# wenet-e2e/wetts

Measured on AMD Instinct MI355X. Metric: audio samples/sec + RTF @22.05 kHz, VITS-Baker, 1/2/4/8 MI355X, higher is better.
Workload: dtype f32

## Files before the change

wetts_amd/csrc/common.h:

```cpp
#pragma once
#include <hip/hip_runtime.h>
#include <stdint.h>
#include <stdio.h>
#include <string>

#include <string.h>

#include "../../include/wetts_hip.h"

namespace wetts {

void set_error(const char* fmt, ...);

#define WETTS_HIP_CHECK(expr)                                                        \
  do {                                                                               \
    hipError_t _e = (expr);                                                          \
    if (_e != hipSuccess) {                                                          \
      ::wetts::set_error("%s failed: %s (%s:%d)", #expr, hipGetErrorString(_e),      \
                         __FILE__, __LINE__);                                        \
      return WETTS_E_HIP;                                                            \
    }                                                                                \
  } while (0)

static inline bool lds_opt_in(const void* kernel, signed char* state) {
  int dev = 0;
  if (hipGetDevice(&dev) != hipSuccess || dev < 0 || dev >= 64) return false;
  if (state[dev] == 0) {
    const hipError_t e = hipFuncSetAttribute(kernel, hipFuncAttributeMaxDynamicSharedMemorySize, 160 * 1024);
    if (e != hipSuccess) (void)hipGetLastError();
    state[dev] = e == hipSuccess ? 1 : -1;
  }
  return state[dev] > 0;
}

#define WETTS_LAUNCH_CHECK()                                                         \
  do {                                                                               \
    hipError_t _e = hipGetLastError();                                               \
    if (_e != hipSuccess) {                                                          \
      ::wetts::set_error("kernel launch failed: %s (%s:%d)", hipGetErrorString(_e),  \
                         __FILE__, __LINE__);                                        \
      return WETTS_E_HIP;                                                            \
    }                                                                                \
  } while (0)

#define WETTS_REQUIRE(cond, ...)        \
  do {                                  \
    if (!(cond)) {                      \
      ::wetts::set_error(__VA_ARGS__);  \
      return WETTS_E_INVALID;           \
    }                                   \
  } while (0)

#define WETTS_TRY(expr)          \
  do {                           \
    int32_t _r = (expr);         \
    if (_r != WETTS_OK) return _r; \
  } while (0)

constexpr int kConvCK = 16;

enum InAct { IN_NONE = 0, IN_LRELU = 1 };
enum OutAct { OUT_NONE = 0, OUT_RELU = 1, OUT_GELU = 2, OUT_GATE = 3 };
__device__ __forceinline__ float wn_gate(float ta, float sa) { return tanhf(ta) * (1.f / (1.f + expf(-sa))); }

__device__ __forceinline__ float div_small_const(float v, float d, float c) {
  const float q = v * c;
  const float r = __builtin_fmaf(-d, q, v);
  return __builtin_fmaf(r, c, q);
}

__device__ __forceinline__ bool mrf_div_fast(float d) { return d == 3.f || d == 2.f; }
__device__ __forceinline__ float mrf_div(float v, float d, float dinv, bool fast) {
  return fast ? div_small_const(v, d, dinv) : v / d;
}

struct ConvParams {
  const float* x;
  int64_t x_bs, x_cs;
  int Cin, Tin;
  int vec_in;
  int in_rev_base;
  int in_act;
  float in_slope;
  const float* in_mask;
  int64_t in_mask_stride;
  const float* wpk;
  const float* bias;
  const float* bias_b;
  int64_t bias_b_stride;
  int M, N;
  int ktaps, dil, pad;
  int off_lo, span;
  int nchunks;
  float* out;
  int64_t o_bs, o_cs;
  int Tout;
  int up_shift;
  int up, up_pad;
  int out_act;
  const float* out_mask;
  int64_t out_mask_stride;
  const float* res;
  int64_t r_bs, r_cs;
  int accum;
  float out_div;
  int B;
  int tag;
  int k_rows_padded;
  const int64_t* lens;
  int len_mul;
  float* wn_h;
  float* wn_skip;
  const float* wn_mask;
  int64_t wn_mask_stride;
  int wn_H, wn_last, wn_first;
};

inline ConvParams conv_io(const float* x, int Cin, int T, float* out, int Cout, int B) {
  ConvParams p;
  memset(&p, 0, sizeof(p));
  p.x = x;
  p.x_bs = (int64_t)Cin * T;
  p.x_cs = T;
  p.Tin = T;
  p.in_rev_base = -1;
  p.in_act = IN_NONE;
  p.in_slope = 0.f;
  p.out = out;
  p.o_bs = (int64_t)Cout * T;
  p.o_cs = T;
  p.Tout = T;
  p.out_act = OUT_NONE;
  p.out_div = 1.f;
  p.B = B;
  return p;
}

struct PackedConv {
  float* wpk = nullptr;
  const float* bias = nullptr;
  int M = 0, Cin = 0, ktaps = 0, dil = 1, pad = 0;
  int up = 0, up_pad = 0;
  int Cout = 0;
  int k_orig = 0;
  int off_lo = 0, span = 0, nchunks = 0;
  int gate_H = 0;
};

int32_t pack_conv_weight(const float* w_dev, const float* bias_dev, int Cout, int Cin, int k,
                         int dil, int pad, int transposed, int up, hipStream_t stream,
                         PackedConv* out, int rev_in = 0, int gate_H = 0);
void free_packed(PackedConv* pc);

int32_t launch_conv(const PackedConv& pc, ConvParams p, hipStream_t stream);
bool pw_gemm_eligible(const PackedConv& pc, const ConvParams& p);
int32_t launch_pw_gemm(const PackedConv& pc, const ConvParams& p, hipStream_t stream, int variant);
int32_t launch_conv_group(const PackedConv* const* pcs, const ConvParams* ps, int n, hipStream_t stream,
                          int* launches = nullptr);

int conv_variant();
void set_conv_variant(int v);
int32_t launch_conv_small(const ConvParams& p, hipStream_t stream, bool* taken);
struct SmallConvScope {
  explicit SmallConvScope(int max_tiles);
  ~SmallConvScope();
  int prev;
};

inline int cdiv(int a, int b) { return (a + b - 1) / b; }
inline int64_t align_up(int64_t v, int64_t a) { return (v + a - 1) / a * a; }

inline int device_cus() {
  static int cus = 0;
  if (cus == 0) {
    int dev = 0, n = 0;
    cus = (hipGetDevice(&dev) == hipSuccess &&
           hipDeviceGetAttribute(&n, hipDeviceAttributeMultiprocessorCount, dev) == hipSuccess && n > 0) ? n : 256;
  }
  return cus;
}

}
```

wetts_amd/csrc/conv_mfma.hip:

```cpp
#include <stdlib.h>

#include "common.h"

namespace wetts {

typedef float f32x16 __attribute__((ext_vector_type(16)));
typedef float f32x4v __attribute__((ext_vector_type(4)));
constexpr int kBufRsrcDword3 = 0x00020000;

__device__ __forceinline__ float lrelu2(float x, float slope) {
  const float m = x * slope;
  float r;
  asm("v_max_f32 %0, %1, %2" : "=v"(r) : "v"(x), "v"(m));
  return r;
}

__global__ void pack_conv_weight_kernel(const float* __restrict__ w, float* __restrict__ out,
                                        int M, int Cin, int Cout, int k, int ktaps, int up,
                                        int transposed, int rev_in, int gate_H, int G, int64_t total) {
  int64_t idx = (int64_t)blockIdx.x * blockDim.x + threadIdx.x;
  if (idx >= total) return;
  int s = (int)(idx & 3);
  int lane = (int)((idx >> 2) & 63);
  int64_t rest = idx >> 8;
// ... 299 lines not shown
  for (int i = 0; i < MB; ++i) a_nxt[i] = abase[i][0];
#pragma unroll
  for (int i = 0; i < MB; ++i) a_alt[i] = a_nxt[i];

  load_chunk(0);
  store_chunk(buf0);
  __syncthreads();

  const int half = lane >> 5;
  const int bcol0 = wn * (32 * NB) + (lane & 31) - p.pad - p.off_lo + sh;
  int g = 0;
  for (int c = 0; c < p.nchunks; ++c) {
    const float* cur = (c & 1) ? buf1 : buf0;
    const bool more = (c + 1) < p.nchunks;
    if (more) load_chunk(c + 1);
    for (int tap = 0; tap < p.ktaps; ++tap) {
      const int coff = bcol0 + tap * p.dil;
#pragma unroll
      for (int hp = 0; hp < 2; ++hp) {
        float4 a_cur[MB];
        ++g;
        if (hp == 0) {
#pragma unroll
          for (int i = 0; i < MB; ++i) a_cur[i] = a_nxt[i];
#pragma unroll
          for (int i = 0; i < MB; ++i) a_alt[i] = abase[i][(int64_t)g * 64];
        } else {
#pragma unroll
          for (int i = 0; i < MB; ++i) a_cur[i] = a_alt[i];
#pragma unroll
          for (int i = 0; i < MB; ++i) a_nxt[i] = abase[i][(int64_t)g * 64];
        }
        __builtin_amdgcn_sched_barrier(0);
        const float* brow0 = cur + (hp * 8 + half) * W + coff;
        float bv[2][NB];
#pragma unroll
        for (int s = 0; s < 4; ++s) {
#pragma unroll
          for (int j = 0; j < NB; ++j) bv[s & 1][j] = brow0[s * 2 * W + 32 * j];
#pragma unroll
          for (int i = 0; i < MB; ++i) {
            const float av = s == 0 ? a_cur[i].x : s == 1 ? a_cur[i].y : s == 2 ? a_cur[i].z
                                                                                 : a_cur[i].w;
#pragma unroll
            for (int j = 0; j < NB; ++j)
              acc[i][j] = __builtin_amdgcn_mfma_f32_32x32x2f32(av, bv[s & 1][j], acc[i][j], 0, 0, 0);
          }
        }
      }
    }
    if (more) store_chunk((c & 1) ? buf0 : buf1);
    __syncthreads();
  }

  const int64_t ob = (int64_t)b * p.o_bs;
  const int64_t rb = (int64_t)b * p.r_bs;
  const float* bb = p.bias_b ? p.bias_b + (int64_t)b * p.bias_b_stride : nullptr;
  const float* omask = p.out_mask ? p.out_mask + (int64_t)b * p.out_mask_stride : nullptr;
  if (EPI == 5) {
    const int gH = p.M >> 1;
#pragma unroll
    for (int i = 0; i < MB; ++i) {
      const int mrow0 = mtile * MT + (wm * MB + i) * 32 + 4 * half;
      float bt[8], bs[8], ut[8], us[8];
#pragma unroll
      for (int q = 0; q < 8; ++q) {
        const int r = 2 * q;
        const int gi = min(mrow0 + (r & 3) + 8 * (r >> 2), p.M - 2) >> 1;
        bt[q] = p.bias ? p.bias[gi] : 0.f;
        bs[q] = p.bias ? p.bias[gH + gi] : 0.f;
        ut[q] = bb ? bb[gi] : 0.f;
        us[q] = bb ? bb[gH + gi] : 0.f;
      }
#pragma unroll
      for (int r = 0; r < 16; r += 2) {
        const int row = mrow0 + (r & 3) + 8 * (r >> 2);
        if (row >= p.M) continue;
        const int gi = row >> 1, q = r >> 1;
        float b0 = bt[q], b1 = bs[q], u0 = ut[q], u1 = us[q];
        if (full_tile) { b0 += u0; b1 += u1; u0 = u1 = 0.f; }
#pragma unroll
        for (int j = 0; j < NB; ++j) {
          const int col = n0 + wn * (32 * NB) + j * 32 + (lane & 31);
          if (col < N)
            p.out[ob + (int64_t)gi * p.o_cs + col] = wn_gate((acc[i][j][r] + b0) + u0, (acc[i][j][r + 1] + b1) + u1);
        }
      }
    }
    return;
  }
  if (EPI != 0 && full_tile) {
    char* obase = reinterpret_cast<char*>(p.out + ob + (int64_t)wrow0 * p.o_cs + wcol0);
    const unsigned ocs4 = (unsigned)p.o_cs * 4u;
    const unsigned olane = (unsigned)(4 * half) * ocs4 + (unsigned)(lane & 31) * 4u;
    float bia[MB][16];
#pragma unroll
    for (int i = 0; i < MB; ++i)
#pragma unroll
      for (int r = 0; r < 16; ++r) bia[i][r] = 0.f;
    if (p.bias) {
      const float* bp = p.bias + wrow0 + 4 * half;
#pragma unroll
      for (int i = 0; i < MB; ++i)
#pragma unroll
        for (int r = 0; r < 16; ++r) bia[i][r] = bp[i * 32 + (r & 3) + 8 * (r >> 2)];
    }
    if (bb) {
      const float* bp = bb + wrow0 + 4 * half;
#pragma unroll
      for (int i = 0; i < MB; ++i)
#pragma unroll
        for (int r = 0; r < 16; ++r) bia[i][r] += bp[i * 32 + (r & 3) + 8 * (r >> 2)];
    }
    float om[NB];
#pragma unroll
    for (int j = 0; j < NB; ++j) om[j] = EPI == 4 ? omask[wcol0 + 32 * j + (lane & 31)] : 1.f;
    auto store_all = [&](auto fin) {
#pragma unroll
      for (int i = 0; i < MB; ++i) {
#pragma unroll
        for (int r = 0; r < 16; ++r) {
          const int rloc = i * 32 + (r & 3) + 8 * (r >> 2);
          const unsigned roff = (unsigned)rloc * ocs4 + olane;
#pragma unroll
          for (int j = 0; j < NB; ++j) {
            float v = fin(acc[i][j][r] + bia[i][r]);
            if (EPI == 4) v *= om[j];
            *reinterpret_cast<float*>(obase + (roff + 128u * j)) = v;
          }
        }
      }
    };
    if (EPI == 2) {
      const float dv = p.out_div, dinv = 1.f / p.out_div;
      if (mrf_div_fast(dv)) store_all([=](float v) { return div_small_const(v, dv, dinv); });
      else store_all([=](float v) { return v / dv; });
    } else {
      store_all([](float v) { return v; });
    }
    return;
  }
  if (EPI == 3) {
    const int sh = p.up_shift, um = p.up - 1;
    char* obase = reinterpret_cast<char*>(p.out + ob);
    const unsigned ocs4 = (unsigned)p.o_cs * 4u;
    float bia[MB][16];
#pragma unroll
    for (int i = 0; i < MB; ++i)
#pragma unroll
      for (int r = 0; r < 16; ++r) {
        const int row = wrow0 + i * 32 + (r & 3) + 8 * (r >> 2) + 4 * half;
        bia[i][r] = (p.bias && row < p.M) ? p.bias[row >> sh] : 0.f;
      }
    if (sh >= 2 && (p.up_pad & 3) == 0 && (Tout & 3) == 0 && (p.M & 3) == 0) {
#pragma unroll
      for (int i = 0; i < MB; ++i) {
#pragma unroll
        for (int q = 0; q < 4; ++q) {
          const int row = wrow0 + i * 32 + 8 * q + 4 * half;
          const int co = row >> sh, ph = row & um;
          const unsigned rowoff = (unsigned)co * ocs4;
#pragma unroll
          for (int j = 0; j < NB; ++j) {
            const int col = wcol0 + 32 * j + (lane & 31);
            const int t = (col << sh) + ph - p.up_pad;
            if (row < p.M && col < N && t >= 0 && t < Tout) {
              f32x4v v;
              v.x = acc[i][j][4 * q] + bia[i][4 * q];
              v.y = acc[i][j][4 * q + 1] + bia[i][4 * q + 1];
              v.z = acc[i][j][4 * q + 2] + bia[i][4 * q + 2];
              v.w = acc[i][j][4 * q + 3] + bia[i][4 * q + 3];
              *reinterpret_cast<f32x4v*>(obase + (rowoff + (unsigned)t * 4u)) = v;
            }
          }
        }
      }
      return;
    }
#pragma unroll
    for (int i = 0; i < MB; ++i) {
#pragma unroll
      for (int r = 0; r < 16; ++r) {
        const int row = wrow0 + i * 32 + (r & 3) + 8 * (r >> 2) + 4 * half;
        const int co = row >> sh, ph = row & um;
        const unsigned rowoff = (unsigned)co * ocs4;
#pragma unroll
        for (int j = 0; j < NB; ++j) {
          const int col = wcol0 + 32 * j + (lane & 31);
          const int t = (col << sh) + ph - p.up_pad;
          if (row < p.M && col < N && t >= 0 && t < Tout)
            *reinterpret_cast<float*>(obase + (rowoff + (unsigned)t * 4u)) = acc[i][j][r] + bia[i][r];
        }
      }
    }
    return;
  }
#pragma unroll
  for (int i = 0; i < MB; ++i) {
    const int mrow0 = mtile * MT + (wm * MB + i) * 32 + 4 * half;
#pragma unroll
    for (int j = 0; j < NB; ++j) {
      const int col = n0 + wn * (32 * NB) + j * 32 + (lane & 31);
      if (col >= N) continue;
#pragma unroll
      for (int r = 0; r < 16; ++r) {
        const int row = mrow0 + (r & 3) + 8 * (r >> 2);
        if (row >= p.M) continue;
        int co = row, t = col;
        if (p.up > 0) {
          co = row / p.up;
          t = col * p.up + (row - co * p.up) - p.up_pad;
          if (t < 0 || t >= Tout) continue;
        }
        float v = acc[i][j][r];
        if (p.bias) v += p.bias[co];
        if (bb) v += bb[co];
        if (p.wn_skip) {
          const int64_t hb = (int64_t)b * p.wn_H * p.Tout + t;
          if (!p.wn_last && row < p.wn_H) {
            float* hp = p.wn_h + hb + (int64_t)row * p.Tout;
            *hp = (*hp + v) * p.wn_mask[(int64_t)b * p.wn_mask_stride + t];
          } else {
            float* sp = p.wn_skip + hb + (int64_t)(p.wn_last ? row : row - p.wn_H) * p.Tout;
            *sp = p.wn_first ? v : *sp + v;
          }
          continue;
        }
        if (p.out_act == OUT_RELU) v = v > 0.f ? v : 0.f;
        if (p.out_act == OUT_GELU) v = 0.5f * v * (1.f + erff(v * 0.70710678118654752f));
        if (omask) v *= omask[t];
        float* dst = p.out + ob + (int64_t)co * p.o_cs + t;
        if (!pre_res) {
          if (p.res) v += p.res[rb + (int64_t)co * p.r_cs + t];
          if (p.accum) v += *dst;
        }
        if (p.out_div != 1.f) v = mrf_div(v, p.out_div, 1.f / p.out_div, mrf_div_fast(p.out_div));
        *dst = v;
      }
    }
  }
}

template <int MB, int NB, int WM, int WN, int EPI = 0, bool MRF = false, bool FAST = false>
__global__ __launch_bounds__(256) __attribute__((amdgpu_waves_per_eu((MB * NB >= 4 && WN < 4) ? 3 : 1)))
void conv_mfma_kernel(const ConvParams p) {
  conv_mfma_body<MB, NB, WM, WN, EPI, FAST>(p, blockIdx.x);
}

constexpr int kConvGroupMax = 3;
struct ConvGroupParams {
  ConvParams p[kConvGroupMax];
  int first[kConvGroupMax + 1];
  int n;
};
template <int MB, int NB, int WM, int WN, int EPI>
__global__ __launch_bounds__(256) __attribute__((amdgpu_waves_per_eu((MB * NB >= 4 && WN < 4) ? 3 : 1)))
void conv_mfma_group_kernel(const ConvGroupParams gp) {
  const int bid = blockIdx.x;
  int j = 0;
  if (gp.n > 1 && bid >= gp.first[1]) j = 1;
  if (gp.n > 2 && bid >= gp.first[2]) j = 2;
  conv_mfma_body<MB, NB, WM, WN, EPI, true>(gp.p[j], bid - gp.first[j]);
}



static bool conv_fast_ok(const ConvParams& p);

static int g_conv_variant = -1;

int conv_variant() {
  if (g_conv_variant < 0) {
    const char* e = getenv("WETTS_CONV_VARIANT");
    g_conv_variant = e ? atoi(e) : 0;
  }
  return g_conv_variant;
}
void set_conv_variant(int v) { g_conv_variant = v; }

template <int MB, int NB, int WM, int WN>
static int32_t launch_cfg(const ConvParams& p, hipStream_t stream) {
  constexpr int MT = 32 * MB * WM, NT = 32 * NB * WN;
  int ntiles = cdiv(p.N, NT), mtiles = cdiv(p.M, MT);
  int64_t blocks = (int64_t)ntiles * mtiles * p.B;
  if (blocks <= 0) return WETTS_OK;
  WETTS_REQUIRE(blocks < (1ll << 31), "conv grid too large");
  const bool fast = conv_fast_ok(p);
  const size_t lds = (size_t)2 * kConvCK *
                     (fast ? (conv_has_fixed_stride(NT) ? conv_fixed_stride(NT) : ((NT + p.span + 3 + 3) & ~3)) : NT + p.span) *
                     sizeof(float);
  const dim3 grid((unsigned)blocks), blk(256);
  const bool plain = p.up == 0 && p.out_act == OUT_NONE && p.out_mask == nullptr && p.wn_skip == nullptr;
  if (p.out_act == OUT_GATE) {
    if (fast)
      hipLaunchKernelGGL((conv_mfma_kernel<MB, NB, WM, WN, 5, false, true>), grid, blk, lds, stream, p);
    else
      hipLaunchKernelGGL((conv_mfma_kernel<MB, NB, WM, WN, 5, false>), grid, blk, lds, stream, p);
  } else if (p.up > 0 && p.up_shift >= 0 && p.out_act == OUT_NONE && !p.out_mask && !p.res && !p.accum &&
      !p.bias_b && p.out_div == 1.f) {
    if (fast)
      hipLaunchKernelGGL((conv_mfma_kernel<MB, NB, WM, WN, 3, false, true>), grid, blk, lds, stream, p);
    else
      hipLaunchKernelGGL((conv_mfma_kernel<MB, NB, WM, WN, 3, false>), grid, blk, lds, stream, p);
  } else if (p.up == 0 && p.out_act == OUT_NONE && p.out_mask && !p.res && !p.accum && p.out_div == 1.f) {
    if (fast)
      hipLaunchKernelGGL((conv_mfma_kernel<MB, NB, WM, WN, 4, false, true>), grid, blk, lds, stream, p);
    else
      hipLaunchKernelGGL((conv_mfma_kernel<MB, NB, WM, WN, 4, false>), grid, blk, lds, stream, p);
  } else if (plain && p.tag && fast) {
    if (p.out_div == 1.f)
      hipLaunchKernelGGL((conv_mfma_kernel<MB, NB, WM, WN, 1, true, true>), grid, blk, lds, stream, p);
    else
      hipLaunchKernelGGL((conv_mfma_kernel<MB, NB, WM, WN, 2, true, true>), grid, blk, lds, stream, p);
  } else if (plain && p.tag) {
    if (p.out_div == 1.f)
      hipLaunchKernelGGL((conv_mfma_kernel<MB, NB, WM, WN, 1, true>), grid, blk, lds, stream, p);
    else
      hipLaunchKernelGGL((conv_mfma_kernel<MB, NB, WM, WN, 2, true>), grid, blk, lds, stream, p);
  } else if (plain && p.out_div == 1.f && fast) {
    hipLaunchKernelGGL((conv_mfma_kernel<MB, NB, WM, WN, 1, false, true>), grid, blk, lds, stream, p);
  } else if (plain && p.out_div == 1.f) {
    hipLaunchKernelGGL((conv_mfma_kernel<MB, NB, WM, WN, 1, false>), grid, blk, lds, stream, p);
  } else if (plain) {
    hipLaunchKernelGGL((conv_mfma_kernel<MB, NB, WM, WN, 2, false>), grid, blk, lds, stream, p);
  } else if (fast) {
    hipLaunchKernelGGL((conv_mfma_kernel<MB, NB, WM, WN, 0, false, true>), grid, blk, lds, stream, p);
  } else {
    hipLaunchKernelGGL((conv_mfma_kernel<MB, NB, WM, WN, 0, false>), grid, blk, lds, stream, p);
  }
  WETTS_LAUNCH_CHECK();
  return WETTS_OK;
}

static int32_t prepare_conv(const PackedConv& pc, ConvParams& p) {
  p.wpk = pc.wpk;
  p.bias = pc.bias;
  p.M = pc.M;
  p.Cin = pc.Cin;
  p.ktaps = pc.ktaps;
  p.dil = pc.dil;
  p.pad = pc.pad;
  p.off_lo = pc.off_lo;
  p.span = pc.span;
  p.nchunks = pc.nchunks;
  p.up = pc.up;
  p.up_pad = pc.up_pad;
  p.up_shift = -1;
  for (int q = 0; q < 16; ++q)
    if (pc.up == (1 << q)) p.up_shift = q;
  WETTS_REQUIRE(pc.wpk != nullptr, "conv weight not packed");
  WETTS_REQUIRE((p.out_act == OUT_GATE) == (pc.gate_H > 0), "gate epilogue and interleaved packing go together");
  WETTS_REQUIRE(p.out_act != OUT_GATE || (!p.res && !p.accum && !p.out_mask && p.out_div == 1.f && !p.wn_skip && pc.up == 0),
                "gate epilogue: plain store only");
  if (pc.ktaps == 1 && pc.up == 0 && p.in_mask && p.in_mask == p.out_mask &&
      p.in_mask_stride == p.out_mask_stride && p.out_act == OUT_NONE)
    p.in_mask = nullptr;
  WETTS_REQUIRE(p.span <= 128, "conv receptive field too wide (span %d > 128)", p.span);
  if (p.up > 0) {
    p.N = p.Tin + p.ktaps - 1;
  } else {
    p.N = p.Tout;
  }
  return WETTS_OK;
}

static bool conv_fast_ok(const ConvParams& p) {
  return p.in_mask == nullptr && p.in_rev_base < 0 && (p.Cin % kConvCK) == 0 && (p.x_cs & 3) == 0 &&
         (p.x_bs & 3) == 0 && (p.Tin & 3) == 0 && p.span <= 125 && (reinterpret_cast<uintptr_t>(p.x) & 15) == 0 &&
         ((int64_t)p.Cin * p.x_cs) < (1ll << 29) && (p.lens == nullptr || (p.len_mul & 3) == 0);
}

template <int MB, int NB, int WM, int WN>
static int32_t launch_group_cfg(ConvGroupParams& gp, int max_span, hipStream_t stream) {
  constexpr int MT = 32 * MB * WM, NT = 32 * NB * WN;
  int64_t total = 0;
  for (int j = 0; j < gp.n; ++j) {
    gp.first[j] = (int)total;
    total += (int64_t)cdiv(gp.p[j].N, NT) * cdiv(gp.p[j].M, MT) * gp.p[j].B;
  }
  gp.first[gp.n] = (int)total;
  WETTS_REQUIRE(total > 0 && total < (1ll << 31), "conv group grid size");
  const size_t lds = (size_t)2 * kConvCK * (conv_has_fixed_stride(NT) ? conv_fixed_stride(NT) : ((NT + max_span + 3 + 3) & ~3)) *
                     sizeof(float);
  hipLaunchKernelGGL((conv_mfma_group_kernel<MB, NB, WM, WN, 1>), dim3((unsigned)total), dim3(256), lds, stream, gp);
  WETTS_LAUNCH_CHECK();
  return WETTS_OK;
}

int32_t launch_conv_group(const PackedConv* const* pcs, const ConvParams* ps, int n, hipStream_t stream,
                          int* launches) {
  if (launches) *launches = n;
  if (n <= 0) return WETTS_OK;
  ConvGroupParams gp;
  memset(&gp, 0, sizeof(gp));
  bool ok = n >= 2 && n <= kConvGroupMax && conv_variant() == 0;
  int order[kConvGroupMax] = {0, 1, 2};
  if (ok) {
    for (int a = 0; a < n; ++a)
      for (int b = a + 1; b < n; ++b)
        if (pcs[order[b]]->ktaps > pcs[order[a]]->ktaps) { int t = order[a]; order[a] = order[b]; order[b] = t; }
  }
  int max_span = 0;
  for (int j = 0; j < n && ok; ++j) {
    gp.p[j] = ps[order[j]];
    WETTS_TRY(prepare_conv(*pcs[order[j]], gp.p[j]));
    const ConvParams& q = gp.p[j];
    ok = q.up == 0 && q.out_act == OUT_NONE && q.out_mask == nullptr && q.out_div == 1.f && q.tag && conv_fast_ok(q) &&
         q.M == gp.p[0].M && q.N == gp.p[0].N && q.B == gp.p[0].B && q.Cin == gp.p[0].Cin && q.lens == gp.p[0].lens;
    if (q.span > max_span) max_span = q.span;
  }
  gp.n = n;
  if (ok) {
    const ConvParams& q = gp.p[0];
    const int64_t cols = (int64_t)q.N * q.B;
    auto nblk = [&](int mt, int nt) { return (int64_t)cdiv(q.M, mt) * cdiv(q.N, nt) * q.B; };
    if (q.M >= 128 && cols >= 4096 && nblk(128, 128) >= 384) {
      if (launches) *launches = 1;
      return launch_group_cfg<1, 4, 4, 1>(gp, max_span, stream);
    }
    if (q.M > 32 && q.M < 128 && cols >= 8192 && nblk(64, 256) >= 384) {
      if (launches) *launches = 1;
      return launch_group_cfg<1, 4, 2, 2>(gp, max_span, stream);
    }
  }
  for (int j = 0; j < n; ++j) WETTS_TRY(launch_conv(*pcs[j], ps[j], stream));
  return WETTS_OK;
}

int32_t launch_conv(const PackedConv& pc, ConvParams p, hipStream_t stream) {
  WETTS_TRY(prepare_conv(pc, p));
  if (conv_variant() == 0 && p.lens == nullptr) {
    bool taken = false;
    WETTS_TRY(launch_conv_small(p, stream, &taken));
    if (taken) return WETTS_OK;
  }
  {
    const int v = conv_variant();
    if ((v == 0 || (v >= 7 && v <= 9)) && pw_gemm_eligible(pc, p)) return launch_pw_gemm(pc, p, stream, v);
  }
  const int64_t cols = (int64_t)p.N * p.B;
  switch (conv_variant()) {
    case 2: return launch_cfg<1, 2, 4, 1>(p, stream);
    case 3: return launch_cfg<1, 4, 2, 2>(p, stream);
    case 4: return launch_cfg<1, 2, 2, 2>(p, stream);
    case 5: return launch_cfg<1, 1, 2, 2>(p, stream);
    case 6: return launch_cfg<1, 4, 4, 1>(p, stream);
    default: break;
  }
  auto nblk = [&](int mt, int nt) { return (int64_t)cdiv(p.M, mt) * cdiv(p.N, nt) * p.B; };
  constexpr int64_t kFill = 384;
  if (p.M >= 128 && cols >= 4096) {
    const int64_t n128 = nblk(128, 128);
    const int kCUs = device_cus();
    if (n128 >= 4 * kCUs) return launch_cfg<1, 4, 4, 1>(p, stream);
    auto cost = [&](int64_t blocks, int area, double eff) {
      return (blocks < kCUs ? 4.0 : 1.0) * (double)((blocks + kCUs - 1) / kCUs) * area / eff;
    };
    const double c128 = cost(n128, 128 * 128, 1.18), c64w = cost(nblk(64, 128), 64 * 128, 1.07),
                 c64 = cost(nblk(64, 64), 64 * 64, 1.0);
    if (c128 <= c64w && c128 <= c64) return launch_cfg<1, 4, 4, 1>(p, stream);
    if (c64w <= c64) return launch_cfg<1, 2, 2, 2>(p, stream);
    return launch_cfg<1, 1, 2, 2>(p, stream);
  }
  if (p.M > 32 && cols >= 8192) {
    if (nblk(64, 256) >= kFill) return launch_cfg<1, 4, 2, 2>(p, stream);
    return launch_cfg<1, 1, 2, 2>(p, stream);
  }
  if (p.M <= 32 && cols >= 8192 && p.ktaps >= 5) return launch_cfg<1, 4, 1, 4>(p, stream);
  if (p.M <= 32 && cols >= 8192) return launch_cfg<1, 2, 1, 4>(p, stream);
  return launch_cfg<1, 1, 2, 2>(p, stream);
}

}
```

wetts_amd/csrc/kernels.h:

```cpp
#pragma once
#include "common.h"

namespace wetts {

int32_t k_embed_mask(const int64_t* ids, const int64_t* lengths, const float* emb, int n_vocab,
                     int B, int H, int T, float* x_out, float* mask_out, int32_t* status,
                     hipStream_t s);

int32_t k_layernorm(const float* a, const float* add, const float* gamma, const float* beta,
                    const float* res, const float* mask, int gelu, int B, int C, int T, float* out,
                    hipStream_t s);

struct DdsFusedParams {
  const float* x;
  float* out;
  const float* mask;
  const float *sep_w[3], *sep_b[3], *n1g[3], *n1b[3], *n2g[3], *n2b[3];
  const float* wpk[3];
  const float* bias[3];
  int B, C, T, G;
};
bool dds_fused_supported(int mode, int C, int Cw, int nchunks, int B, int T);
int32_t k_dds_fused(DdsFusedParams p, hipStream_t s);
int32_t k_dwconv(const float* x, const float* mask, const float* w, const float* bias, int k,
                 int dil, int B, int C, int T, float* out, hipStream_t s, int Tvalid = 0);

int32_t k_cond_linear(const float* g, const float* W, const float* bias, int B, int Cout, int K,
                      float* out, hipStream_t s);

int32_t k_gather_rows(const int64_t* idx, const float* table, int n_rows, int B, int C, float* out,
                      int32_t* status, hipStream_t s);

int32_t k_add_bias_b(float* x, const float* v, int B, int C, int T, hipStream_t s);
int32_t k_add_bias_b_mask(float* x, const float* v, const float* mask, int B, int C, int T,
                          hipStream_t s);
int32_t k_scale(const float* a, float scale, int64_t n, float* out, hipStream_t s);

int32_t k_convflow_pre(const float* z, int ch0, const float* w, const float* bias, const float* g,
                       int B, int C, int T, float* out, hipStream_t s);

int32_t k_spline_inverse(float* z, int ch0, int ch1, const float* h, const float* mask,
                         int num_bins, float tail_bound, float inv_sqrt_div, int B, int T,
                         int32_t* status, hipStream_t s);

int32_t k_affine_reverse(const float* z, int ch, const float* m, const float* logs, int param_idx,
                         const float* mask, int B, int T, float* logw, hipStream_t s);

int32_t k_gate(const float* a, int B, int H, int T, float* out, hipStream_t s);

int32_t k_wn_update(const float* rs, float* h, float* skip, const float* mask, int last, int first,
                    int B, int H, int T, hipStream_t s);

int32_t k_coupling_flip(const float* xin, const float* m, const float* mask, int B, int C, int T,
                        float* out, hipStream_t s);

int32_t k_conv_post_tanh(const float* x, const float* w, int k, int B, int C, int T, float* out,
                         hipStream_t s, const int64_t* lens = nullptr, int len_mul = 0);

int32_t k_durations_to_lengths(const float* logw, const float* mask, float length_scale, int B,
                               int T, float* w_ceil, float* cum, int64_t* y_lengths,
                               int32_t* status, hipStream_t s);

int32_t k_frame_index(const float* cum, const int64_t* y_lengths, int B, int Tx, int Ty,
                      int32_t* frame2phone, float* y_mask, hipStream_t s);
int32_t k_expand_prior(const float* stats, const int32_t* frame2phone, const float* eps,
                       int64_t eps_bs, int64_t eps_cs, float noise_scale, int B, int C, int Tx, int Ty, float* m_exp,
                       float* logs_exp, float* z_p, hipStream_t s);
int32_t k_attn_path(const int32_t* frame2phone, int B, int Tx, int Ty, float* attn, hipStream_t s);

int32_t k_audio_to_int16(const float* audio, const int64_t* lengths, int B, int64_t L, int16_t* pcm,
                         hipStream_t s);

int32_t k_vocos_pad(const float* z, int64_t z_bs, int64_t z_cs, const float* mask,
                    int64_t mask_stride, int B, int C, int L, float* out, hipStream_t s, int Fs = 0);
int32_t k_vocos_spec(const float* spec, int B, int half, int F, float* ri, hipStream_t s, int64_t ri_bs = 0);
int32_t k_istft_basis(int n_fft, float* w, hipStream_t s, double inv_scale = 0.0);
bool k_convnext_dwln(const float* x, const float* w, const float* wb, const float* gamma, const float* beta, int B, int C,
                     int T, int Tvalid, float* out, hipStream_t s, int32_t* rc);
int32_t k_istft_ola(const float* frames, int B, int n_fft, int hop, int F, float* audio,
                    hipStream_t s, int Fs = 0, int envelope = 1);
int32_t k_scale_rows(const float* a, const float* scale, int rows, int cols, float* out,
                     hipStream_t s);

int32_t k_flip_half(const float* x, const float* mask, int B, int C, int T, float* x0, float* x0m,
                    hipStream_t s);
int32_t k_mono_split(const float* x, const float* mask, int B, int C, int T, float sc, float* x0, float* x0m,
                     hipStream_t s);
int32_t k_mono_coupling(const float* x, const float* m, const float* mask, int B, int C, int T, float sc, float* out,
                        hipStream_t s);
int32_t k_coupling_fwd_flip(const float* x, const float* m, const float* mask, int B, int C, int T, float* out,
                            hipStream_t s);
int32_t k_mono_coupling_fwd(const float* x, const float* m, const float* mask, int B, int C, int T, int residual,
                            float* out, hipStream_t s);
int32_t k_seq_mask(const int64_t* lengths, int B, int T_in, int Tp, float* mask, float* mask_out, hipStream_t s);
int32_t k_posterior_sample(const float* stats, const float* eps, const float* mask, int B, int C, int T, int Tp,
                           float* z, float* m_out, float* logs_out, hipStream_t s);
int32_t k_copy_rows(const float* src, int64_t src_stride, int cols_src, float* dst, int64_t dst_stride, int cols_dst,
                    int64_t rows, hipStream_t s);
int32_t k_add(const float* a, const float* b, int64_t n, float* out, hipStream_t s);

int32_t k_rel_attention(const float* q, const float* k, const float* v, int64_t qkv_batch_stride,
                        const float* mask, const float* emb_rel_k, const float* emb_rel_v,
                        int window, int B, int n_heads, int dk, int T, float* scores, float* out,
                        hipStream_t s);

int64_t attn_score_elems(int window, int dk, int B, int n_heads, int T);

int32_t k_randn(float* out, int64_t n, uint64_t seed, uint64_t offset, hipStream_t s);
int32_t k_mask_rows(const float* x, const float* mask, int B, int C, int T, float* out,
                    hipStream_t s);

int32_t k_mas(const float* neg_cent, const int32_t* t_ys, const int32_t* t_xs, int B, int Ty,
              int Tx, int32_t* path, float* values, hipStream_t s);

int32_t k_align_scores(const float* z_p, const float* stats, int B, int I, int Tx, int Ty, float* neg_cent,
                       hipStream_t s);
int32_t k_align_lengths(const int64_t* x_lengths, const int64_t* y_lengths, int B, int Tx, int Ty, int32_t* t_xs,
                        int32_t* t_ys, int32_t* status, hipStream_t s);
int32_t k_path_to_durations(const int32_t* path, const int32_t* t_ys, const int32_t* t_xs, int B, int Tx, int Ty,
                            float* w, float* cum, int32_t* frame2phone, float* attn, hipStream_t s);
int32_t k_counts_to_lengths(const int64_t* counts, const float* mask, int B, int T, float* w_ceil, float* cum,
                            int64_t* y_lengths, int32_t* status, hipStream_t s);

}
```

wetts_amd/csrc/kernels.hip:

```cpp
#include "kernels.h"

namespace wetts {

static inline dim3 grid1d(int64_t n, int threads) {
  return dim3((unsigned)((n + threads - 1) / threads));
}

__global__ void embed_mask_kernel(const int64_t* __restrict__ ids,
                                  const int64_t* __restrict__ lengths,
                                  const float* __restrict__ emb, int n_vocab, int B, int H, int T,
                                  float scale, float* __restrict__ x_out,
                                  float* __restrict__ mask_out, int32_t* __restrict__ status) {
  int64_t idx = (int64_t)blockIdx.x * blockDim.x + threadIdx.x;
  int64_t total = (int64_t)B * H * T;
  if (idx >= total) return;
  int t = (int)(idx % T);
  int c = (int)((idx / T) % H);
  int b = (int)(idx / ((int64_t)T * H));
  bool valid = (int64_t)t < lengths[b];
  float v = 0.f;
  if (valid) {
    int64_t id = ids[(int64_t)b * T + t];
    if (id < 0 || id >= n_vocab) {
      if (status && c == 0) atomicOr(status, WETTS_STATUS_PHONE_ID_RANGE);
// ... 499 lines not shown
int32_t k_affine_reverse(const float* z, int ch, const float* m, const float* logs, int param_idx,
                         const float* mask, int B, int T, float* logw, hipStream_t s) {
  if (B * T == 0) return WETTS_OK;
  hipLaunchKernelGGL(affine_reverse_kernel, grid1d((int64_t)B * T, 256), dim3(256), 0, s, z, ch, m,
                     logs, param_idx, mask, B, T, logw);
  WETTS_LAUNCH_CHECK();
  return WETTS_OK;
}

__global__ void gate_kernel(const float* __restrict__ a, int B, int H, int T,
                            float* __restrict__ out) {
  int64_t idx = (int64_t)blockIdx.x * blockDim.x + threadIdx.x;
  int64_t total = (int64_t)B * H * T;
  if (idx >= total) return;
  int64_t ht = (int64_t)H * T;
  int64_t b = idx / ht, r = idx % ht;
  float ta = a[b * 2 * ht + r];
  float sa = a[b * 2 * ht + ht + r];
  out[idx] = tanhf(ta) * (1.f / (1.f + expf(-sa)));
}

int32_t k_gate(const float* a, int B, int H, int T, float* out, hipStream_t s) {
  int64_t n = (int64_t)B * H * T;
  if (n == 0) return WETTS_OK;
  hipLaunchKernelGGL(gate_kernel, grid1d(n, 256), dim3(256), 0, s, a, B, H, T, out);
  WETTS_LAUNCH_CHECK();
  return WETTS_OK;
}

__global__ void wn_update_kernel(const float* __restrict__ rs, float* __restrict__ h,
                                 float* __restrict__ skip, const float* __restrict__ mask, int last,
                                 int first, int B, int H, int T) {
  int64_t idx = (int64_t)blockIdx.x * blockDim.x + threadIdx.x;
  int64_t total = (int64_t)B * H * T;
  if (idx >= total) return;
  int64_t ht = (int64_t)H * T;
  int64_t b = idx / ht, r = idx % ht;
  int t = (int)(r % T);
  float sk;
  if (!last) {
    float res = rs[b * 2 * ht + r];
    sk = rs[b * 2 * ht + ht + r];
    h[idx] = (h[idx] + res) * mask[b * T + t];
  } else {
    sk = rs[idx];
  }
  skip[idx] = first ? sk : skip[idx] + sk;
}

int32_t k_wn_update(const float* rs, float* h, float* skip, const float* mask, int last, int first,
                    int B, int H, int T, hipStream_t s) {
  int64_t n = (int64_t)B * H * T;
  if (n == 0) return WETTS_OK;
  hipLaunchKernelGGL(wn_update_kernel, grid1d(n, 256), dim3(256), 0, s, rs, h, skip, mask, last,
                     first, B, H, T);
  WETTS_LAUNCH_CHECK();
  return WETTS_OK;
}

__global__ void coupling_flip_kernel(const float* __restrict__ xin, const float* __restrict__ m,
                                     const float* __restrict__ mask, int B, int C, int T,
                                     float* __restrict__ out) {
  int64_t idx = (int64_t)blockIdx.x * blockDim.x + threadIdx.x;
  int64_t total = (int64_t)B * C * T;
  if (idx >= total) return;
  int t = (int)(idx % T);
  int c = (int)((idx / T) % C);
  int b = (int)(idx / ((int64_t)T * C));
  const int half = C / 2;
  float v = xin[((int64_t)b * C + (C - 1 - c)) * T + t];
  if (c >= half) v = (v - m[((int64_t)b * half + (c - half)) * T + t]) * mask[(int64_t)b * T + t];
  out[idx] = v;
}

int32_t k_coupling_flip(const float* xin, const float* m, const float* mask, int B, int C, int T,
                        float* out, hipStream_t s) {
  int64_t n = (int64_t)B * C * T;
  if (n == 0) return WETTS_OK;
  hipLaunchKernelGGL(coupling_flip_kernel, grid1d(n, 256), dim3(256), 0, s, xin, m, mask, B, C, T,
                     out);
  WETTS_LAUNCH_CHECK();
  return WETTS_OK;
}

__global__ __launch_bounds__(256) void conv_post_tanh_kernel(const float* __restrict__ x,
                                                             const float* __restrict__ w, int k,
                                                             int B, int C, int T,
                                                             float* __restrict__ out,
                                                             const int64_t* __restrict__ lens, int len_mul) {
  extern __shared__ float wsh[];
  for (int i = threadIdx.x; i < C * k; i += blockDim.x) wsh[i] = w[i];
  __syncthreads();
  const int per_b = (T + 3) / 4;
  int64_t idx = (int64_t)blockIdx.x * blockDim.x + threadIdx.x;
  if (idx >= (int64_t)B * per_b) return;
  const int b = (int)(idx / per_b);
  const int t0 = (int)(idx % per_b) * 4;
  const int pad = (k - 1) / 2;
  float acc[4] = {0.f, 0.f, 0.f, 0.f};
  const float* xb = x + (int64_t)b * C * T;
  const int Tb = lens ? min((int)lens[b] * len_mul, T) : T;
  if (t0 >= Tb) {
#pragma unroll
    for (int o = 0; o < 4; ++o)
      if (t0 + o < T) out[(int64_t)b * T + t0 + o] = 0.f;
    return;
  }
  if (k == 7 && (T & 3) == 0 && t0 >= 4 && t0 + 8 <= Tb && (C & 3) == 0 &&
      (reinterpret_cast<uintptr_t>(xb) & 15) == 0) {
    for (int c = 0; c < C; c += 4) {
      float4 v[4][3];
#pragma unroll
      for (int u = 0; u < 4; ++u) {
        const float4* xr4 = reinterpret_cast<const float4*>(xb + (int64_t)(c + u) * T + (t0 - 4));
        v[u][0] = xr4[0];
        v[u][1] = xr4[1];
        v[u][2] = xr4[2];
      }
#pragma unroll
      for (int u = 0; u < 4; ++u) {
        const float raw[10] = {v[u][0].y, v[u][0].z, v[u][0].w, v[u][1].x, v[u][1].y,
                               v[u][1].z, v[u][1].w, v[u][2].x, v[u][2].y, v[u][2].z};
        float win[10];
#pragma unroll
        for (int i = 0; i < 10; ++i) win[i] = raw[i] > 0.f ? raw[i] : raw[i] * 0.01f;
#pragma unroll
        for (int j = 0; j < 7; ++j) {
          const float wv = wsh[(c + u) * 7 + j];
#pragma unroll
          for (int o = 0; o < 4; ++o) acc[o] += wv * win[o + j];
        }
      }
    }
  } else
  for (int c = 0; c < C; ++c) {
    const float* xr = xb + (int64_t)c * T;
    float win[4 + 15];
    for (int i = 0; i < 3 + k; ++i) {
      int tt = t0 - pad + i;
      float v = (tt >= 0 && tt < Tb) ? xr[tt] : 0.f;
      win[i] = v > 0.f ? v : v * 0.01f;
    }
    for (int j = 0; j < k; ++j) {
      float wv = wsh[c * k + j];
#pragma unroll
      for (int o = 0; o < 4; ++o) acc[o] += wv * win[o + j];
    }
  }
#pragma unroll
  for (int o = 0; o < 4; ++o)
    if (t0 + o < T) out[(int64_t)b * T + t0 + o] = (t0 + o < Tb) ? tanhf(acc[o]) : 0.f;
}

template <int K>
__global__ __launch_bounds__(256) void conv_post_tanh_small_kernel(const float* __restrict__ x,
                                                                   const float* __restrict__ w, int B,
                                                                   int C, int T, float* __restrict__ out) {
  constexpr int TL = 32, CG = 8, MAXC = 8;
  __shared__ float red[CG][TL + 1];
  const int tl = threadIdx.x % TL, cg = threadIdx.x / TL;
  const int tblocks = (T + TL - 1) / TL;
  const int b = blockIdx.x / tblocks;
  const int t = (blockIdx.x % tblocks) * TL + tl;
  constexpr int pad = (K - 1) / 2;
  const float* xb = x + (int64_t)b * C * T;
  float win[MAXC][K], wv[MAXC][K];
#pragma unroll
  for (int j = 0; j < MAXC; ++j) {
    const int c = cg + CG * j;
    const int cc = c < C ? c : 0;
#pragma unroll
    for (int i = 0; i < K; ++i) {
      const int tt = t - pad + i;
      const bool ok = c < C && tt >= 0 && tt < T;
      win[j][i] = xb[(int64_t)cc * T + (ok ? tt : 0)];
      wv[j][i] = ok ? w[cc * K + i] : 0.f;
    }
  }
  float acc = 0.f;
#pragma unroll
  for (int j = 0; j < MAXC; ++j)
#pragma unroll
    for (int i = 0; i < K; ++i) {
      const float v = win[j][i];
      acc += wv[j][i] * (v > 0.f ? v : v * 0.01f);
    }
  red[cg][tl] = acc;
  __syncthreads();
  if (cg == 0 && t < T) {
    float tot = 0.f;
#pragma unroll
    for (int q = 0; q < CG; ++q) tot += red[q][tl];
    out[(int64_t)b * T + t] = tanhf(tot);
  }
}

int32_t k_conv_post_tanh(const float* x, const float* w, int k, int B, int C, int T, float* out,
                         hipStream_t s, const int64_t* lens, int len_mul) {
  WETTS_REQUIRE(k <= 15, "conv_post kernel size %d unsupported", k);
  int64_t n = (int64_t)B * ((T + 3) / 4);
  if (n == 0) return WETTS_OK;
  if (k == 7 && C <= 64 && n <= 64 * 256 && !lens) {
    hipLaunchKernelGGL(conv_post_tanh_small_kernel<7>, dim3((unsigned)(B * cdiv(T, 32))), dim3(256), 0, s, x, w,
                       B, C, T, out);
    WETTS_LAUNCH_CHECK();
    return WETTS_OK;
  }
  hipLaunchKernelGGL(conv_post_tanh_kernel, grid1d(n, 256), dim3(256), (size_t)C * k * 4, s, x, w,
                     k, B, C, T, out, lens, len_mul);
  WETTS_LAUNCH_CHECK();
  return WETTS_OK;
}

__global__ __launch_bounds__(64) void durations_kernel(const float* __restrict__ logw,
                                                       const float* __restrict__ mask,
                                                       float length_scale, int B, int T,
                                                       float* __restrict__ w_ceil,
                                                       float* __restrict__ cum,
                                                       int64_t* __restrict__ y_lengths,
                                                       int32_t* __restrict__ status) {
  const int b = blockIdx.x, lane = threadIdx.x;
  float carry = 0.f;
  for (int t0 = 0; t0 < T; t0 += 64) {
    int t = t0 + lane;
    float wc = 0.f;
    if (t < T) {
      float w = expf(logw[(int64_t)b * T + t]) * mask[(int64_t)b * T + t] * length_scale;
      wc = ceilf(w);
      w_ceil[(int64_t)b * T + t] = wc;
    }
    float v = wc;
#pragma unroll
    for (int off = 1; off < 64; off <<= 1) {
      float n = __shfl_up(v, off, 64);
      if (lane >= off) v += n;
    }
    v += carry;
    if (t < T) cum[(int64_t)b * T + t] = v;
    carry = __shfl(v, 63, 64);
  }
  if (lane == 0) {
    float tot = carry < 1.f ? 1.f : carry;
    if (!(tot <= 9.0e15f)) {
      if (status) atomicOr(status, WETTS_STATUS_DURATION_NONFINITE);
      tot = 1.f;
    }
    y_lengths[b] = (int64_t)tot;
  }
}

int32_t k_durations_to_lengths(const float* logw, const float* mask, float length_scale, int B,
                               int T, float* w_ceil, float* cum, int64_t* y_lengths,
                               int32_t* status, hipStream_t s) {
  if (B == 0) return WETTS_OK;
  hipLaunchKernelGGL(durations_kernel, dim3(B), dim3(64), 0, s, logw, mask, length_scale, B, T,
                     w_ceil, cum, y_lengths, status);
  WETTS_LAUNCH_CHECK();
  return WETTS_OK;
}

__global__ void frame_index_kernel(const float* __restrict__ cum,
                                   const int64_t* __restrict__ y_lengths, int B, int Tx, int Ty,
                                   int32_t* __restrict__ f2p, float* __restrict__ y_mask) {
  int idx = blockIdx.x * blockDim.x + threadIdx.x;
  if (idx >= B * Ty) return;
  int ty = idx % Ty, b = idx / Ty;
  bool valid = (int64_t)ty < y_lengths[b];
  int res = -1;
  if (valid) {
    const float* cr = cum + (int64_t)b * Tx;
    int lo = 0, hi = Tx;
    float fy = (float)ty;
    while (lo < hi) {
      int mid = (lo + hi) >> 1;
      if (cr[mid] > fy) hi = mid; else lo = mid + 1;
    }
    if (lo < Tx) res = lo;
  }
  f2p[idx] = res;
  y_mask[idx] = valid ? 1.f : 0.f;
}

int32_t k_frame_index(const float* cum, const int64_t* y_lengths, int B, int Tx, int Ty,
                      int32_t* frame2phone, float* y_mask, hipStream_t s) {
  if (B * Ty == 0) return WETTS_OK;
  hipLaunchKernelGGL(frame_index_kernel, grid1d((int64_t)B * Ty, 256), dim3(256), 0, s, cum,
                     y_lengths, B, Tx, Ty, frame2phone, y_mask);
  WETTS_LAUNCH_CHECK();
  return WETTS_OK;
}

__global__ void expand_prior_kernel(const float* __restrict__ stats,
                                    const int32_t* __restrict__ f2p, const float* __restrict__ eps,
                                    int64_t eps_bs, int64_t eps_cs, float noise_scale, int B, int C, int Tx, int Ty,
                                    float* __restrict__ m_exp, float* __restrict__ logs_exp,
                                    float* __restrict__ z_p) {
  int64_t idx = (int64_t)blockIdx.x * blockDim.x + threadIdx.x;
  int64_t total = (int64_t)B * C * Ty;
  if (idx >= total) return;
  int ty = (int)(idx % Ty);
  int c = (int)((idx / Ty) % C);
  int b = (int)(idx / ((int64_t)Ty * C));
  int tx = f2p[(int64_t)b * Ty + ty];
  float m = 0.f, ls = 0.f;
  if (tx >= 0) {
    m = stats[((int64_t)b * 2 * C + c) * Tx + tx];
    ls = stats[((int64_t)b * 2 * C + C + c) * Tx + tx];
  }
  if (m_exp) m_exp[idx] = m;
  if (logs_exp) logs_exp[idx] = ls;
  const float e = eps[(int64_t)b * eps_bs + (int64_t)c * eps_cs + ty];
  z_p[idx] = m + e * expf(ls) * noise_scale;
}

int32_t k_expand_prior(const float* stats, const int32_t* frame2phone, const float* eps,
                       int64_t eps_bs, int64_t eps_cs, float noise_scale, int B, int C, int Tx, int Ty, float* m_exp,
                       float* logs_exp, float* z_p, hipStream_t s) {
  int64_t n = (int64_t)B * C * Ty;
  if (n == 0) return WETTS_OK;
  hipLaunchKernelGGL(expand_prior_kernel, grid1d(n, 256), dim3(256), 0, s, stats, frame2phone, eps,
                     eps_bs, eps_cs, noise_scale, B, C, Tx, Ty, m_exp, logs_exp, z_p);
  WETTS_LAUNCH_CHECK();
  return WETTS_OK;
}

__global__ void attn_path_kernel(const int32_t* __restrict__ f2p, int B, int Tx, int Ty,
                                 float* __restrict__ attn) {
  int64_t idx = (int64_t)blockIdx.x * blockDim.x + threadIdx.x;
  int64_t total = (int64_t)B * Ty * Tx;
  if (idx >= total) return;
  int tx = (int)(idx % Tx);
  int64_t bty = idx / Tx;
  attn[idx] = (f2p[bty] == tx) ? 1.f : 0.f;
}

int32_t k_attn_path(const int32_t* frame2phone, int B, int Tx, int Ty, float* attn, hipStream_t s) {
  int64_t n = (int64_t)B * Ty * Tx;
  if (n == 0) return WETTS_OK;
  hipLaunchKernelGGL(attn_path_kernel, grid1d(n, 256), dim3(256), 0, s, frame2phone, B, Tx, Ty,
                     attn);
  WETTS_LAUNCH_CHECK();
  return WETTS_OK;
}

__global__ __launch_bounds__(256) void audio_to_int16_kernel(const float* __restrict__ audio,
                                                             const int64_t* __restrict__ lengths,
                                                             int64_t L, int16_t* __restrict__ pcm) {
  __shared__ float red[4];
  const int b = blockIdx.x;
  const float* a = audio + (int64_t)b * L;
  int64_t n = lengths ? lengths[b] : L;
  if (n > L) n = L;
  float mx = 0.f;
  for (int64_t i = threadIdx.x; i < n; i += blockDim.x) mx = fmaxf(mx, fabsf(a[i]));
#pragma unroll
// ... 428 lines not shown
```

Baseline: 52.49 million.

## Add cost-model tile choice for upsampling convs and staged-tile conv_post kernel

Moves conv tile selection into a reusable function and gives transposed/upsampling convs their own cost model across 128x128, 128x64 and 64x128 tiles, instead of always taking 128x128 when the block count is large. It also adds an LDS double-buffered conv_post+tanh kernel that stages four channels at a time with halos. That kernel only runs when variant==2, and no caller in view passes that value. The vectorized upsample store now also checks output alignment, which guards against misaligned float4 writes.

```diff
diff --git a/wetts_amd/csrc/common.h b/wetts_amd/csrc/common.h
--- a/wetts_amd/csrc/common.h
+++ b/wetts_amd/csrc/common.h
@@ -160,6 +160,7 @@
 
 int conv_variant();
 void set_conv_variant(int v);
+int conv_tile_choice(int M, int N, int B, int ktaps, int up, int cus);
 int32_t launch_conv_small(const ConvParams& p, hipStream_t stream, bool* taken);
 struct SmallConvScope {
   explicit SmallConvScope(int max_tiles);
diff --git a/wetts_amd/csrc/conv_mfma.hip b/wetts_amd/csrc/conv_mfma.hip
--- a/wetts_amd/csrc/conv_mfma.hip
+++ b/wetts_amd/csrc/conv_mfma.hip
@@ -475,7 +475,8 @@
         const int row = wrow0 + i * 32 + (r & 3) + 8 * (r >> 2) + 4 * half;
         bia[i][r] = (p.bias && row < p.M) ? p.bias[row >> sh] : 0.f;
       }
-    if (sh >= 2 && (p.up_pad & 3) == 0 && (Tout & 3) == 0 && (p.M & 3) == 0) {
+    if (sh >= 2 && (p.up_pad & 3) == 0 && (Tout & 3) == 0 && (p.M & 3) == 0 && (p.o_cs & 3) == 0 &&
+        (reinterpret_cast<uintptr_t>(obase) & 15) == 0) {
 #pragma unroll
       for (int i = 0; i < MB; ++i) {
 #pragma unroll
@@ -589,6 +590,8 @@
 
 
 static bool conv_fast_ok(const ConvParams& p);
+
+constexpr double kUpEff128 = 1.18, kUpEff128n = 1.10, kUpEff64w = 1.07;
 
 static int g_conv_variant = -1;
 
@@ -761,7 +764,6 @@
     const int v = conv_variant();
     if ((v == 0 || (v >= 7 && v <= 9)) && pw_gemm_eligible(pc, p)) return launch_pw_gemm(pc, p, stream, v);
   }
-  const int64_t cols = (int64_t)p.N * p.B;
   switch (conv_variant()) {
     case 2: return launch_cfg<1, 2, 4, 1>(p, stream);
     case 3: return launch_cfg<1, 4, 2, 2>(p, stream);
@@ -770,28 +772,47 @@
     case 6: return launch_cfg<1, 4, 4, 1>(p, stream);
     default: break;
   }
-  auto nblk = [&](int mt, int nt) { return (int64_t)cdiv(p.M, mt) * cdiv(p.N, nt) * p.B; };
+  switch (conv_tile_choice(p.M, p.N, p.B, p.ktaps, p.up, device_cus())) {
+    case 128128: return launch_cfg<1, 4, 4, 1>(p, stream);
+    case 128064: return launch_cfg<1, 2, 4, 1>(p, stream);
+    case 64256: return launch_cfg<1, 4, 2, 2>(p, stream);
+    case 64128: return launch_cfg<1, 2, 2, 2>(p, stream);
+    case 32512: return launch_cfg<1, 4, 1, 4>(p, stream);
+    case 32256: return launch_cfg<1, 2, 1, 4>(p, stream);
+    default: return launch_cfg<1, 1, 2, 2>(p, stream);
+  }
+}
+
+int conv_tile_choice(int M, int N, int B, int ktaps, int up, int cus) {
+  const int64_t cols = (int64_t)N * B;
+  auto nblk = [&](int mt, int nt) { return (int64_t)cdiv(M, mt) * cdiv(N, nt) * B; };
   constexpr int64_t kFill = 384;
-  if (p.M >= 128 && cols >= 4096) {
+  if (M >= 128 && cols >= 4096) {
     const int64_t n128 = nblk(128, 128);
-    const int kCUs = device_cus();
-    if (n128 >= 4 * kCUs) return launch_cfg<1, 4, 4, 1>(p, stream);
+    const int kCUs = cus;
     auto cost = [&](int64_t blocks, int area, double eff) {
       return (blocks < kCUs ? 4.0 : 1.0) * (double)((blocks + kCUs - 1) / kCUs) * area / eff;
     };
+    if (up > 0) {
+      const double u128 = cost(n128, 128 * 128, kUpEff128), u128n = cost(nblk(128, 64), 128 * 64, kUpEff128n),
+                   u64w = cost(nblk(64, 128), 64 * 128, kUpEff64w);
+      if (u128 <= u128n && u128 <= u64w) return 128128;
+      return u128n <= u64w ? 128064 : 64128;
+    }
+    if (n128 >= 4 * kCUs) return 128128;
     const double c128 = cost(n128, 128 * 128, 1.18), c64w = cost(nblk(64, 128), 64 * 128, 1.07),
                  c64 = cost(nblk(64, 64), 64 * 64, 1.0);
-    if (c128 <= c64w && c128 <= c64) return launch_cfg<1, 4, 4, 1>(p, stream);
-    if (c64w <= c64) return launch_cfg<1, 2, 2, 2>(p, stream);
-    return launch_cfg<1, 1, 2, 2>(p, stream);
-  }
-  if (p.M > 32 && cols >= 8192) {
-    if (nblk(64, 256) >= kFill) return launch_cfg<1, 4, 2, 2>(p, stream);
-    return launch_cfg<1, 1, 2, 2>(p, stream);
-  }
-  if (p.M <= 32 && cols >= 8192 && p.ktaps >= 5) return launch_cfg<1, 4, 1, 4>(p, stream);
-  if (p.M <= 32 && cols >= 8192) return launch_cfg<1, 2, 1, 4>(p, stream);
-  return launch_cfg<1, 1, 2, 2>(p, stream);
-}
-
-}
+    if (c128 <= c64w && c128 <= c64) return 128128;
+    if (c64w <= c64) return 64128;
+    return 64064;
+  }
+  if (M > 32 && cols >= 8192) {
+    if (nblk(64, 256) >= kFill) return 64256;
+    return 64064;
+  }
+  if (M <= 32 && cols >= 8192 && ktaps >= 5) return 32512;
+  if (M <= 32 && cols >= 8192) return 32256;
+  return 64064;
+}
+
+}
diff --git a/wetts_amd/csrc/kernels.h b/wetts_amd/csrc/kernels.h
--- a/wetts_amd/csrc/kernels.h
+++ b/wetts_amd/csrc/kernels.h
@@ -55,7 +55,7 @@
                         float* out, hipStream_t s);
 
 int32_t k_conv_post_tanh(const float* x, const float* w, int k, int B, int C, int T, float* out,
-                         hipStream_t s, const int64_t* lens = nullptr, int len_mul = 0);
+                         hipStream_t s, const int64_t* lens = nullptr, int len_mul = 0, int variant = 0);
 
 int32_t k_durations_to_lengths(const float* logw, const float* mask, float length_scale, int B,
                                int T, float* w_ceil, float* cum, int64_t* y_lengths,
diff --git a/wetts_amd/csrc/kernels.hip b/wetts_amd/csrc/kernels.hip
--- a/wetts_amd/csrc/kernels.hip
+++ b/wetts_amd/csrc/kernels.hip
@@ -675,6 +675,90 @@
     if (t0 + o < T) out[(int64_t)b * T + t0 + o] = (t0 + o < Tb) ? tanhf(acc[o]) : 0.f;
 }
 
+constexpr int kPostTW = 1024, kPostCG = 4, kPostW = kPostTW + 8;
+__global__ __launch_bounds__(256) void conv_post_tanh_tile_kernel(const float* __restrict__ x,
+                                                                  const float* __restrict__ w, int B, int C, int T,
+                                                                  float* __restrict__ out,
+                                                                  const int64_t* __restrict__ lens, int len_mul) {
+  __shared__ __attribute__((aligned(16))) float sm[2][kPostCG][kPostW];
+  const int tid = threadIdx.x;
+  const int tiles = (T + kPostTW - 1) / kPostTW;
+  const int b = blockIdx.x / tiles;
+  const int tile0 = (blockIdx.x % tiles) * kPostTW;
+  const int t0 = tile0 + 4 * tid;
+  const int Tb = lens ? min((int)lens[b] * len_mul, T) : T;
+  float* ob = out + (int64_t)b * T;
+  if (tile0 >= Tb) {
+    if (t0 < T) *reinterpret_cast<float4*>(ob + t0) = float4{0.f, 0.f, 0.f, 0.f};
+    return;
+  }
+  const float* xb = x + (int64_t)b * C * T;
+  auto piece = [&](const float* row, int t) {
+    float4 v = float4{0.f, 0.f, 0.f, 0.f};
+    if (t >= 0 && t < Tb) {
+      v = *reinterpret_cast<const float4*>(row + t);
+      if (t + 4 > Tb) {
+        if (t + 1 >= Tb) v.y = 0.f;
+        if (t + 2 >= Tb) v.z = 0.f;
+        v.w = 0.f;
+      }
+    }
+    return v;
+  };
+  auto lr = [](float4 v) {
+    v.x = v.x > 0.f ? v.x : v.x * 0.01f;
+    v.y = v.y > 0.f ? v.y : v.y * 0.01f;
+    v.z = v.z > 0.f ? v.z : v.z * 0.01f;
+    v.w = v.w > 0.f ? v.w : v.w * 0.01f;
+    return v;
+  };
+  const int hu = tid & 3, ht = tid < 4 ? tile0 - 4 : tile0 + kPostTW, hcol = tid < 4 ? 0 : kPostTW + 4;
+  float4 own[kPostCG], halo;
+  auto load_group = [&](int c) {
+#pragma unroll
+    for (int u = 0; u < kPostCG; ++u) own[u] = piece(xb + (int64_t)(c + u) * T, t0);
+    if (tid < 8) halo = piece(xb + (int64_t)(c + hu) * T, ht);
+  };
+  auto store_group = [&](int buf) {
+#pragma unroll
+    for (int u = 0; u < kPostCG; ++u) *reinterpret_cast<float4*>(&sm[buf][u][4 + 4 * tid]) = lr(own[u]);
+    if (tid < 8) *reinterpret_cast<float4*>(&sm[buf][hu][hcol]) = lr(halo);
+  };
+  load_group(0);
+  store_group(0);
+  __syncthreads();
+  float acc[4] = {0.f, 0.f, 0.f, 0.f};
+  for (int c = 0; c < C; c += kPostCG) {
+    const int buf = (c / kPostCG) & 1;
+    const bool more = c + kPostCG < C;
+    if (more) load_group(c + kPostCG);
+    if (t0 < Tb) {
+#pragma unroll
+      for (int u = 0; u < kPostCG; ++u) {
+        const float4* r4 = reinterpret_cast<const float4*>(&sm[buf][u][4 * tid]);
+        const float4 a = r4[0], m = r4[1], z = r4[2];
+        const float win[10] = {a.y, a.z, a.w, m.x, m.y, m.z, m.w, z.x, z.y, z.z};
+#pragma unroll
+        for (int j = 0; j < 7; ++j) {
+          const float wv = w[(c + u) * 7 + j];
+#pragma unroll
+          for (int o = 0; o < 4; ++o) acc[o] += wv * win[o + j];
+        }
+      }
+    }
+    if (more) store_group(buf ^ 1);
+    __syncthreads();
+  }
+  if (t0 < T) {
+    float4 r;
+    r.x = t0 < Tb ? tanhf(acc[0]) : 0.f;
+    r.y = t0 + 1 < Tb ? tanhf(acc[1]) : 0.f;
+    r.z = t0 + 2 < Tb ? tanhf(acc[2]) : 0.f;
+    r.w = t0 + 3 < Tb ? tanhf(acc[3]) : 0.f;
+    *reinterpret_cast<float4*>(ob + t0) = r;
+  }
+}
+
 template <int K>
 __global__ __launch_bounds__(256) void conv_post_tanh_small_kernel(const float* __restrict__ x,
                                                                    const float* __restrict__ w, int B,
@@ -719,11 +803,21 @@
 }
 
 int32_t k_conv_post_tanh(const float* x, const float* w, int k, int B, int C, int T, float* out,
-                         hipStream_t s, const int64_t* lens, int len_mul) {
+                         hipStream_t s, const int64_t* lens, int len_mul, int variant) {
   WETTS_REQUIRE(k <= 15, "conv_post kernel size %d unsupported", k);
   int64_t n = (int64_t)B * ((T + 3) / 4);
   if (n == 0) return WETTS_OK;
-  if (k == 7 && C <= 64 && n <= 64 * 256 && !lens) {
+  const int64_t tiles = (int64_t)B * cdiv(T, kPostTW);
+  const bool tile_ok = k == 7 && (T & 3) == 0 && (C % kPostCG) == 0 && tiles < (1ll << 31) &&
+                       ((reinterpret_cast<uintptr_t>(x) | reinterpret_cast<uintptr_t>(out)) & 15) == 0;
+  WETTS_REQUIRE(variant != 2 || tile_ok, "conv_post: the staged-tile kernel does not take this shape");
+  if (tile_ok && variant == 2) {
+    hipLaunchKernelGGL(conv_post_tanh_tile_kernel, dim3((unsigned)tiles), dim3(256), 0, s, x, w, B, C, T, out, lens,
+                       len_mul);
+    WETTS_LAUNCH_CHECK();
+    return WETTS_OK;
+  }
+  if (variant == 0 && k == 7 && C <= 64 && n <= 64 * 256 && !lens) {
     hipLaunchKernelGGL(conv_post_tanh_small_kernel<7>, dim3((unsigned)(B * cdiv(T, 32))), dim3(256), 0, s, x, w,
                        B, C, T, out);
     WETTS_LAUNCH_CHECK();
```

After: 52.39 million. About the same (-0.2%).
